# thiviyanT/torch-rgcn

Measured on AMD Instinct MI355X. Metric: edges/s/GPU (fwd+bwd) 2-layer RGCN, 1M nodes/10M edges/50 rels, h=16, higher is better.
Workload: dtype f32; 1 GPU; S1: N=1000000 nodes, E=10000000 base triples, R0=50 relations (layer R=101), M=21000000 messages/layer, hidden=16, 2 NC layers (horizontal, vertical), fwd+bwd, learnable X

## Files before the change

### torch-rgcn_amd/csrc/rgcn_bwd_own.hip

```cpp
#include <stdlib.h>
#include <string.h>

#include <algorithm>

#include "rgcn_device.h"

namespace {

constexpr int OWN_REC = 176;
constexpr int OWN_REC_ROWS = 128;
constexpr int OWN_REC_HDR = 160;
constexpr int OWN_LDS_MAX = 160 * 1024;
#ifndef RGCN_OWN_NW
#define RGCN_OWN_NW 16
#define RGCN_OWN_K 8
#define RGCN_OWN_U 2
#endif
constexpr int OWN_NW = RGCN_OWN_NW;
constexpr int OWN_K = RGCN_OWN_K;
constexpr int OWN_U = RGCN_OWN_U;
constexpr int OWN_MAX_ROWS = (OWN_LDS_MAX - OWN_NW * BW_SCR2 * 4 - 64) / 192;

#define OWN_DW_CASE(I)                                                                                             \
  if constexpr (I < K) {                                                                                           \
    if (lr == I) {                                                                                                 \
      _Pragma("unroll") for (int t4 = 0; t4 < 4; ++t4)                                                             \
        accw[I] = __builtin_amdgcn_mfma_f32_16x16x4f32(a[t4], b[t4], accw[I], 0, 0, 0);                            \
    }                                                                                                              \
    asm volatile("" : "+s"(lr));                                                                                   \
  }

size_t bwd_own_lds(int rows, bool packed = false) { return (size_t)rows * 192 + (size_t)OWN_NW * BW_SCR2 * 4 + 64 + (packed ? PK_LDS : 0); }
constexpr int OWN_MAX_ROWS_PK = (OWN_LDS_MAX - OWN_NW * BW_SCR2 * 4 - 64 - PK_LDS) / 192;

template <bool RELU, int NW, int K, int ABL = 0, bool BF = false, bool PK = false>
__global__ __launch_bounds__(64 * NW) void bwd_own_d16_kernel(
    const float *__restrict__ G, const float *__restrict__ X, const float *__restrict__ Wtp, float *__restrict__ dX,
    float *__restrict__ dWout, const char *__restrict__ rec, const int *__restrict__ gptr, int gstride, int shared_rel, int n_tiles,
    int tile_rows, int n_dst, float *__restrict__ dbias, int n_src, const int *__restrict__ unit_rel) {
  constexpr int U = OWN_U, NT = 64 * NW;
  constexpr int TQ = (OWN_MAX_ROWS * 4 + NT - 1) / NT;
  static_assert(K <= 9, "dw_add lists nine accumulator cases");
  extern __shared__ __attribute__((aligned(16))) char lds[];
  const int tid = threadIdx.x;
  const int wave = __builtin_amdgcn_readfirstlane(tid >> 6), lane = tid & 63;
  const unsigned xt_off = (unsigned)tile_rows * 128u;
  const unsigned xs_off = (unsigned)tile_rows * 192u;
  float4 *dxz = reinterpret_cast<float4 *>(lds);
  const double2 *dxd2 = reinterpret_cast<const double2 *>(lds);
  float4 *xt4 = reinterpret_cast<float4 *>(lds + xt_off);
  float *xs = reinterpret_cast<float *>(lds + xs_off) + wave * BW_SCR2;
  int *ctr = reinterpret_cast<int *>(lds + xs_off + (unsigned)NW * BW_SCR2 * 4u);
  const bool takes = shared_rel >= 0 && __builtin_amdgcn_readfirstlane(unit_rel[wave * K + K - 1]) == shared_rel;
  auto take = [&]() {
    int v = 0;
    if (lane == 0) v = __hip_atomic_fetch_add(ctr, U, __ATOMIC_RELAXED, __HIP_MEMORY_SCOPE_WORKGROUP);
    return __builtin_amdgcn_readfirstlane(v);
  };
  auto ranges = [&](int tt, int &a, int &b, int &sa, int &sb) {
    const int *g = gptr + (size_t)tt * gstride;
    a = __builtin_amdgcn_readfirstlane(g[wave]);
    b = __builtin_amdgcn_readfirstlane(g[wave + 1]);
    sa = sb = 0;
    if (takes) {
      sa = __builtin_amdgcn_readfirstlane(g[NW]);
      sb = __builtin_amdgcn_readfirstlane(g[NW + 1]);
    }
  };

  int t = blockIdx.x;
  int row0 = t * tile_rows;
  int nrows = min(tile_rows, n_dst - row0);
  int c0, c1, s0, s1;
  ranges(t, c0, c1, s0, s1);
  if (tid == 0) lds_st(ctr, 0);
  const float *dict = reinterpret_cast<const float *>(ctr + 16);
  if constexpr (PK)
    for (int i = tid; i <= PK_DICT; i += NT) ctr[16 + i] = i < PK_DICT ? reinterpret_cast<const int *>(rec)[i] : 0;
  float4 gs = make_float4(0.f, 0.f, 0.f, 0.f);
  const long long g_n4 = dbias ? (long long)n_src * 4 : 0, g_step = (long long)gridDim.x * NT;
  long long g_i = (long long)blockIdx.x * NT + tid;
#pragma unroll
  for (int q = 0; q < TQ; ++q) {
    const int idx = tid + q * NT;
    if (idx < tile_rows * 4) {
      float4 x0 = make_float4(0.f, 0.f, 0.f, 0.f);
      if (idx < nrows * 4) {
        if constexpr (BF) x0 = bf16x4_widen(reinterpret_cast<const uint2 *>(X)[(size_t)row0 * 4 + idx]);
        else x0 = reinterpret_cast<const float4 *>(X + (size_t)row0 * 16)[idx];
      }
      xt4[idx] = x0;
    }
  }
  for (int i = tid; i < tile_rows * 8; i += NT) dxz[i] = make_float4(0.f, 0.f, 0.f, 0.f);
  __syncthreads();

  const int m = lane & 15, k = lane >> 4;
  const unsigned kofs = (unsigned)k << 4;
  const unsigned dx_lane = (unsigned)m * 8u;
  const unsigned xrd = xt_off + (unsigned)m * 4u;
  float *xs_wr = xs + m * 16 + 4 * ((k + (m >> 2)) & 3);
  const float *xs_rd = xs + (4 * k) * 16 + 4 * (((m >> 2) + k) & 3) + (m & 3);
  const unsigned slot_lane = (unsigned)m * 8u;
  const unsigned rows_lane = (unsigned)OWN_REC_ROWS + (unsigned)k * 8u;
  const unsigned w_lane = (unsigned)lane * 16u;

  f32x4 accw[K];
#pragma unroll
  for (int i = 0; i < K; ++i) accw[i] = f32x4{0.f, 0.f, 0.f, 0.f};
  auto dw_add = [&](int lr, const float (&a)[4], const float (&b)[4]) {
    OWN_DW_CASE(0) OWN_DW_CASE(1) OWN_DW_CASE(2) OWN_DW_CASE(3) OWN_DW_CASE(4) OWN_DW_CASE(5) OWN_DW_CASE(6) OWN_DW_CASE(7) OWN_DW_CASE(8)
  };

  uint2 sl_n[U], rw_n[U];
  int hd_n[U];
  auto request_idx = [&](int c, int last) {
#pragma unroll
    for (int j = 0; j < U; ++j) {
      const int cc = min(c + j, last);
      if constexpr (PK) {
        const char *r = rec + PK_DICT_BYTES + (size_t)cc * PK_REC;
        sl_n[j].x = *reinterpret_cast<const unsigned *>(r + (unsigned)m * 4u);
        rw_n[j] = *reinterpret_cast<const uint2 *>(r + ((unsigned)PK_REC_ROWS + (unsigned)k * 8u));
      } else {
      const char *r = rec + (size_t)cc * OWN_REC;
      sl_n[j] = *reinterpret_cast<const uint2 *>(r + slot_lane);
      rw_n[j] = *reinterpret_cast<const uint2 *>(r + rows_lane);
      hd_n[j] = *reinterpret_cast<const int *>(r + OWN_REC_HDR);
      }
    }
  };
  if (c0 < c1) request_idx(c0, c1 - 1);

  for (;;) {
    int c = c0, last = c1 - 1;
    bool sh = false;
    if (c > last && s0 < s1) {
      sh = true;
      c = s0 + take();
      last = s1 - 1;
      if (c <= last) request_idx(c, last);
    }
    while (c <= last) {
      unsigned w0_[U];
      uint2 rw_[U];
      float v_[U];
      int hd_[U];
      float4 g_[U], w_[U];
#pragma unroll
      for (int j = 0; j < U; ++j) {
        if constexpr (PK) {
          w0_[j] = (sl_n[j].x >> 2) & 0xFFFFFFC0u;
          rw_[j] = rw_n[j];
          v_[j] = dict[(c + j <= last) ? sl_n[j].x & 0xFFu : (unsigned)PK_DICT];
          hd_[j] = pk_header(__builtin_amdgcn_readfirstlane(rw_n[j].x), __builtin_amdgcn_readfirstlane(rw_n[j].y));
        } else {
        w0_[j] = sl_n[j].x;
        rw_[j] = rw_n[j];
        v_[j] = (c + j <= last) ? __builtin_bit_cast(float, sl_n[j].y) : 0.f;
        hd_[j] = __builtin_amdgcn_readfirstlane(hd_n[j]);
        }
      }
      if constexpr (PK) {
#pragma unroll
        for (int j = 0; j < U; ++j) asm volatile("" : "+v"(w0_[j]));
      } else {
#pragma unroll
      for (int j = 0; j < U; ++j) asm volatile("" : "+v"(w0_[j]), "+v"(v_[j]));
      }
      __builtin_amdgcn_sched_barrier(0);
#pragma unroll
      for (int j = 0; j < U; ++j) {
        if constexpr (BF) {
          g_[j] = bf16x4_widen(*reinterpret_cast<const uint2 *>(reinterpret_cast<const char *>(G) + ((w0_[j] >> 1) | (kofs >> 1))));
        } else {
          const unsigned og = w0_[j] | kofs;
          g_[j] = *reinterpret_cast<const float4 *>(reinterpret_cast<const char *>(G) + og);
        }
        w_[j] = *reinterpret_cast<const float4 *>(reinterpret_cast<const char *>(Wtp) + (size_t)(hd_[j] & 0xFFFF) * 1024 + w_lane);
      }
      __builtin_amdgcn_sched_barrier(0);
      {
        int cn = c + U, lastn = last;
        if (sh || (cn > last && s0 < s1)) {
          sh = true;
          cn = s0 + take();
          lastn = s1 - 1;
        }
        if (cn <= lastn) request_idx(cn, lastn);
        c = cn;
        last = lastn;
      }
      __builtin_amdgcn_sched_barrier(0);
      if (ABL & 16) {
#pragma unroll
        for (int j = 0; j < U; ++j) asm volatile("" :: "v"(g_[j].x), "v"(g_[j].y), "v"(g_[j].z), "v"(g_[j].w), "v"(w_[j].x), "v"(w_[j].w), "v"(rw_[j].x), "v"(rw_[j].y), "v"(v_[j]));
        continue;
      }
      f32x4 sc[U], acc[U];
#pragma unroll
      for (int j = 0; j < U; ++j) {
        sc[j] = f32x4{g_[j].x * v_[j], g_[j].y * v_[j], g_[j].z * v_[j], g_[j].w * v_[j]};
        acc[j] = f32x4{0.f, 0.f, 0.f, 0.f};
      }
#pragma unroll
      for (int j = 0; j < U; ++j) acc[j] = __builtin_amdgcn_mfma_f32_16x16x4f32(sc[j][0], w_[j].x, acc[j], 0, 0, 0);
#pragma unroll
      for (int j = 0; j < U; ++j) acc[j] = __builtin_amdgcn_mfma_f32_16x16x4f32(sc[j][1], w_[j].y, acc[j], 0, 0, 0);
#pragma unroll
      for (int j = 0; j < U; ++j) acc[j] = __builtin_amdgcn_mfma_f32_16x16x4f32(sc[j][2], w_[j].z, acc[j], 0, 0, 0);
#pragma unroll
      for (int j = 0; j < U; ++j) acc[j] = __builtin_amdgcn_mfma_f32_16x16x4f32(sc[j][3], w_[j].w, acc[j], 0, 0, 0);
      unsigned ro[U][4];
#pragma unroll
      for (int j = 0; j < U; ++j) {
        ro[j][0] = rw_[j].x & 0xFFFFu;
        ro[j][1] = rw_[j].x >> 16;
        ro[j][2] = rw_[j].y & 0xFFFFu;
        ro[j][3] = rw_[j].y >> 16;
        if constexpr (PK) {
#pragma unroll
          for (int e = 0; e < 4; ++e) ro[j][e] &= 0xFFC0u;
        }
      }
#pragma unroll
      for (int h = 0; h < U && !(ABL & 2); h += 2) {
        constexpr int P = 2;
        float bv[P][4], av[P][4];
#pragma unroll
        for (int jj = 0; jj < P; ++jj) {
          const int j = h + jj;
          if (j >= U) break;
          asm volatile("" ::: "memory");
          *reinterpret_cast<f32x4 *>(xs_wr) = sc[j];
          asm volatile("" ::: "memory");
#pragma unroll
          for (int t4 = 0; t4 < 4; ++t4) bv[jj][t4] = xs_rd[16 * t4];
#pragma unroll
          for (int t4 = 0; t4 < 4; ++t4) av[jj][t4] = *reinterpret_cast<const float *>(lds + (xrd + ro[j][t4]));
          asm volatile("" ::: "memory");
        }
#pragma unroll
        for (int jj = 0; jj < P; ++jj) {
          if (h + jj >= U) break;
          dw_add((int)((unsigned)hd_[h + jj] >> 16), av[jj], bv[jj]);
        }
      }
#pragma unroll
      for (int j = 0; j < U && !(ABL & 8); ++j)
#pragma unroll
        for (int e = 0; e < 4; ++e)
          __hip_atomic_fetch_add(static_cast<double *>(__builtin_assume_aligned(lds + (dx_lane + 2u * ro[j][e]), 8)), (double)acc[j][e], __ATOMIC_RELAXED,
                                 __HIP_MEMORY_SCOPE_WORKGROUP);
      __builtin_amdgcn_sched_barrier(0);
    }
    const int tn = t + (int)gridDim.x;
    int c0n = 0, c1n = 0, s0n = 0, s1n = 0, row0n = 0, nrn = 0;
    float4 xn[TQ];
#pragma unroll
    for (int q = 0; q < TQ; ++q) xn[q] = make_float4(0.f, 0.f, 0.f, 0.f);
    if (tn < n_tiles) {
      row0n = tn * tile_rows;
      nrn = min(tile_rows, n_dst - row0n);
      ranges(tn, c0n, c1n, s0n, s1n);
#pragma unroll
      for (int q = 0; q < TQ; ++q)
        if (tid + q * NT < nrn * 4) {
          if constexpr (BF) {
            const uint2 u = reinterpret_cast<const uint2 *>(X)[(size_t)row0n * 4 + tid + q * NT];
            xn[q] = make_float4(__uint_as_float(u.x), __uint_as_float(u.y), 0.f, 0.f);
          } else {
            xn[q] = reinterpret_cast<const float4 *>(X + (size_t)row0n * 16)[tid + q * NT];
          }
        }
      if (c0n < c1n) request_idx(c0n, c1n - 1);
    }
    float4 gn = make_float4(0.f, 0.f, 0.f, 0.f);
    if (g_i < g_n4) {
      if constexpr (BF) gn = bf16x4_widen(reinterpret_cast<const uint2 *>(G)[g_i]);
      else gn = reinterpret_cast<const float4 *>(G)[g_i];
    }
    g_i += g_step;
    lds_barrier();
    gs.x += gn.x; gs.y += gn.y; gs.z += gn.z; gs.w += gn.w;
#pragma unroll
    for (int q = 0; q < TQ; ++q) asm volatile("" : "+v"(xn[q].x), "+v"(xn[q].y), "+v"(xn[q].z), "+v"(xn[q].w));
#pragma unroll
    for (int q = 0; q < TQ; ++q) {
      const int idx = tid + q * NT;
      if (idx < nrows * 4) {
        const double2 d0 = dxd2[2 * idx], d1 = dxd2[2 * idx + 1];
        float4 a = make_float4((float)d0.x, (float)d0.y, (float)d1.x, (float)d1.y);
        if (RELU) {
          const float4 x = xt4[idx];
          a.x = x.x > 0.f ? a.x : 0.f; a.y = x.y > 0.f ? a.y : 0.f; a.z = x.z > 0.f ? a.z : 0.f; a.w = x.w > 0.f ? a.w : 0.f;
        }
        if constexpr (BF) reinterpret_cast<uint2 *>(dX)[(size_t)row0 * 4 + idx] = bf16x4_round(a);
        else reinterpret_cast<float4 *>(dX + (size_t)row0 * 16)[idx] = a;
      }
    }
    if (tn >= n_tiles) break;
    if (tid == 0) lds_st(ctr, 0);
#pragma unroll
    for (int q = 0; q < TQ; ++q) {
      const int idx = tid + q * NT;
      if (idx < tile_rows * 4) {
        dxz[2 * idx] = make_float4(0.f, 0.f, 0.f, 0.f);
        dxz[2 * idx + 1] = make_float4(0.f, 0.f, 0.f, 0.f);
        if constexpr (BF) xt4[idx] = bf16x4_widen(uint2{__float_as_uint(xn[q].x), __float_as_uint(xn[q].y)});
        else xt4[idx] = xn[q];
      }
    }
    lds_barrier();
    t = tn; row0 = row0n; nrows = nrn; c0 = c0n; c1 = c1n; s0 = s0n; s1 = s1n;
  }
  if (dbias) {
    for (; g_i < g_n4; g_i += g_step) {
      float4 gn;
      if constexpr (BF) gn = bf16x4_widen(reinterpret_cast<const uint2 *>(G)[g_i]);
      else gn = reinterpret_cast<const float4 *>(G)[g_i];
      gs.x += gn.x; gs.y += gn.y; gs.z += gn.z; gs.w += gn.w;
    }
#pragma unroll
    for (int sft = 4; sft < 64; sft <<= 1) {
      gs.x += __shfl_xor(gs.x, sft); gs.y += __shfl_xor(gs.y, sft); gs.z += __shfl_xor(gs.z, sft); gs.w += __shfl_xor(gs.w, sft);
    }
    __syncthreads();
    if (lane < 4) *reinterpret_cast<float4 *>(xs + 4 * lane) = gs;
    __syncthreads();
    if (tid < 16) {
      float a = 0.f;
      const float *all = reinterpret_cast<const float *>(lds + xs_off);
      for (int i = 0; i < NW; ++i) a += all[i * BW_SCR2 + tid];
      atomicAdd(dbias + tid, a);
    }
  }
  if (shared_rel >= 0) {
    __syncthreads();
    *reinterpret_cast<f32x4 *>(xs + 4 * lane) = takes ? accw[K - 1] : f32x4{0.f, 0.f, 0.f, 0.f};
    __syncthreads();
    if (wave == 0) {
      const float *all = reinterpret_cast<const float *>(lds + xs_off) + 4 * lane;
      f32x4 a = f32x4{0.f, 0.f, 0.f, 0.f};
      for (int i = 0; i < NW; ++i) a += *reinterpret_cast<const f32x4 *>(all + i * BW_SCR2);
      float *o = dWout + (size_t)shared_rel * 256 + (4 * k) * 16 + m;
      atomicAdd(o, a[0]);
      atomicAdd(o + 16, a[1]);
      atomicAdd(o + 32, a[2]);
      atomicAdd(o + 48, a[3]);
    }
  }
#pragma unroll
  for (int li = 0; li < K; ++li) {
    const int r = __builtin_amdgcn_readfirstlane(unit_rel[wave * K + li]);
    if (r >= 0 && !(takes && li == K - 1)) {
      float *o = dWout + (size_t)r * 256 + (4 * k) * 16 + m;
      atomicAdd(o, accw[li][0]);
      atomicAdd(o + 16, accw[li][1]);
      atomicAdd(o + 32, accw[li][2]);
      atomicAdd(o + 48, accw[li][3]);
    }
  }
}

#undef OWN_DW_CASE

}

extern "C" int32_t rgcn_bwd_own_waves(void) { return OWN_NW; }
extern "C" int32_t rgcn_bwd_own_units(void) { return OWN_NW * OWN_K; }
extern "C" int32_t rgcn_bwd_own_max_rows(void) { return OWN_MAX_ROWS; }
extern "C" int32_t rgcn_bwd_blk_packed_max_rows(int32_t owner) { return owner ? OWN_MAX_ROWS_PK : rgcn_spmm_blk_max_rows(); }

static bool own_groups_ok(const int32_t *own_ptr, const int32_t *group_ptr, int32_t shared_rel, int64_t n_tiles, int32_t R) {
  if (!group_ptr) return own_ptr && shared_rel < 0;
  return shared_rel >= 0 && shared_rel < R && n_tiles * (int64_t)(OWN_NW + 1) < INT32_MAX;
}

extern "C" int rgcn_bwd_own_f32(const float *G, const float *X, const float *Wt_packed, float *dX, float *dW, const void *rec,
                                const int32_t *own_ptr, const int32_t *group_ptr, int32_t shared_rel, const int32_t *unit_rel, int64_t n_tiles,
                                int32_t tile_rows, int64_t n_dst, int32_t R, int32_t flags, float *dbias, int64_t n_src, void *stream) {
  if (!G || !X || !Wt_packed || !dX || !dW || !rec || !unit_rel || n_tiles <= 0 || tile_rows <= 0 || n_dst <= 0 || R <= 0 ||
      R > 0xFFFF || n_dst > INT32_MAX || n_tiles * (int64_t)OWN_NW >= INT32_MAX || !own_groups_ok(own_ptr, group_ptr, shared_rel, n_tiles, R)) {
    rgcn_set_error("bwd_own: bad argument");
    return RGCN_EINVAL;
  }
  const bool packed = (flags & RGCN_F_PACKED_REC) != 0;
  if (tile_rows > (packed ? OWN_MAX_ROWS_PK : OWN_MAX_ROWS)) {
    rgcn_set_error("bwd_own: tiles of at most %d rows (got %d)", packed ? OWN_MAX_ROWS_PK : OWN_MAX_ROWS, tile_rows);
    return RGCN_EUNSUPPORTED;
  }
  if (n_src <= 0 || n_src >= (int64_t(1) << 26)) {
    rgcn_set_error("bwd_own: the records address G rows as src << 6 in 32 bits: 0 < n_src < 2^26");
    return RGCN_EINVAL;
  }
  hipStream_t st = (hipStream_t)stream;
  int dev = 0, n_cu = 0;
  HIP_TRY(launch_device(&dev, &n_cu));
  HIP_TRY(zero_dw_dbias_async(dW, (size_t)R, dbias, st));
  const size_t lds = bwd_own_lds(tile_rows, packed);
  const unsigned n_blocks = (unsigned)std::min<int64_t>(n_tiles, n_cu);
  auto launch = [&](auto k) -> hipError_t {
    constexpr auto kern = decltype(k)::value;
    hipError_t e = allow_lds<kern>(dev, lds, OWN_LDS_MAX);
    if (e != hipSuccess) return e;
    hipLaunchKernelGGL(kern, dim3(n_blocks), dim3(64 * OWN_NW), lds, st, G, X, Wt_packed, dX, dW, static_cast<const char *>(rec), group_ptr ? group_ptr : own_ptr,
                       group_ptr ? OWN_NW + 1 : OWN_NW, group_ptr ? shared_rel : -1, (int)n_tiles, tile_rows, (int)n_dst, dbias, (int)n_src, unit_rel);
    return hipGetLastError();
  };
#ifdef RGCN_ABLATIONS
  {
    const int ABLV = rgcn_option_value(RGCN_OPT_BWD_ABL);
    if (packed) { rgcn_set_error("bwd_own (ablation library): wide records only"); return RGCN_EUNSUPPORTED; }
    if (ABLV == 2) HIP_TRY(launch(kern_c<bwd_own_d16_kernel<false, OWN_NW, OWN_K, 2>>));
    else if (ABLV == 8) HIP_TRY(launch(kern_c<bwd_own_d16_kernel<false, OWN_NW, OWN_K, 8>>));
    else if (ABLV == 16) HIP_TRY(launch(kern_c<bwd_own_d16_kernel<false, OWN_NW, OWN_K, 16>>));
    else HIP_TRY(launch(kern_c<bwd_own_d16_kernel<false, OWN_NW, OWN_K, 0>>));
    return RGCN_OK;
  }
#endif
  if (packed && (flags & RGCN_F_RELU)) HIP_TRY(launch(kern_c<bwd_own_d16_kernel<true, OWN_NW, OWN_K, 0, false, true>>));
  else if (packed) HIP_TRY(launch(kern_c<bwd_own_d16_kernel<false, OWN_NW, OWN_K, 0, false, true>>));
  else if (flags & RGCN_F_RELU) HIP_TRY(launch(kern_c<bwd_own_d16_kernel<true, OWN_NW, OWN_K>>));
  else HIP_TRY(launch(kern_c<bwd_own_d16_kernel<false, OWN_NW, OWN_K>>));
  return RGCN_OK;
}

extern "C" int rgcn_bwd_own_bf16(const uint16_t *G, const uint16_t *X, const float *Wt_packed, uint16_t *dX, float *dW, const void *rec,
                                 const int32_t *own_ptr, const int32_t *group_ptr, int32_t shared_rel, const int32_t *unit_rel, int64_t n_tiles,
                                 int32_t tile_rows, int64_t n_dst, int32_t R, int32_t flags, float *dbias, int64_t n_src, void *stream) {
  if (!G || !X || !Wt_packed || !dX || !dW || !rec || !unit_rel || n_tiles <= 0 || tile_rows <= 0 || n_dst <= 0 || R <= 0 ||
      R > 0xFFFF || n_dst > INT32_MAX || n_tiles * (int64_t)OWN_NW >= INT32_MAX || n_src <= 0 || n_src >= (int64_t(1) << 26) || (flags & ~RGCN_F_PACKED_REC) != 0 ||
      !own_groups_ok(own_ptr, group_ptr, shared_rel, n_tiles, R)) {
    rgcn_set_error("bwd_own_bf16: bad argument (the records address G rows as src << 6 in 32 bits: n_src < 2^26; no flags)");
    return RGCN_EINVAL;
  }
  const bool packed = (flags & RGCN_F_PACKED_REC) != 0;
  if (tile_rows > (packed ? OWN_MAX_ROWS_PK : OWN_MAX_ROWS)) {
    rgcn_set_error("bwd_own_bf16: tiles of at most %d rows (got %d)", packed ? OWN_MAX_ROWS_PK : OWN_MAX_ROWS, tile_rows);
    return RGCN_EUNSUPPORTED;
  }
  hipStream_t st = (hipStream_t)stream;
  int dev = 0, n_cu = 0;
  HIP_TRY(launch_device(&dev, &n_cu));
  HIP_TRY(zero_dw_dbias_async(dW, (size_t)R, dbias, st));
  const size_t lds = bwd_own_lds(tile_rows, packed);
  const unsigned n_blocks = (unsigned)std::min<int64_t>(n_tiles, n_cu);
  auto launch = [&](auto k) -> hipError_t {
    constexpr auto kern = decltype(k)::value;
    hipError_t e = allow_lds<kern>(dev, lds, OWN_LDS_MAX);
    if (e != hipSuccess) return e;
    hipLaunchKernelGGL(kern, dim3(n_blocks), dim3(64 * OWN_NW), lds, st, reinterpret_cast<const float *>(G), reinterpret_cast<const float *>(X),
                       Wt_packed, reinterpret_cast<float *>(dX), dW, static_cast<const char *>(rec), group_ptr ? group_ptr : own_ptr,
                       group_ptr ? OWN_NW + 1 : OWN_NW, group_ptr ? shared_rel : -1, (int)n_tiles, tile_rows, (int)n_dst, dbias, (int)n_src, unit_rel);
    return hipGetLastError();
  };
  if (packed) HIP_TRY(launch(kern_c<bwd_own_d16_kernel<false, OWN_NW, OWN_K, 0, true, true>>));
  else HIP_TRY(launch(kern_c<bwd_own_d16_kernel<false, OWN_NW, OWN_K, 0, true>>));
  return RGCN_OK;
}
```

### torch-rgcn_amd/torch_rgcn/graph.py

```python
import numpy as np
import torch

from . import _native, routes

_LDS_WAVE_FLOATS = 2048


def pick_tile_rows(width, n_rows=None):
    ld = (max(1, width) + 3) & ~3
    env = routes.get("tile_rows")
    if env:
        return max(1, min(int(env), 4096 // ld))
    rows = max(1, min(128, _LDS_WAVE_FLOATS // ld))
    if n_rows is not None and n_rows < rows * 2048:
        rows = max(min(rows, 8), min(rows, n_rows // 2048))
    return int(rows)


_MAX_CELLS = 2 ** 34
_SOFTWIN_MIN_CHUNKS = 4
_OWN_MAX_IMBALANCE = 1.25


class RelGraph:
    def __init__(self, triples_plus, val, num_nodes, num_rels, device):
        self.num_nodes, self.num_rels = int(num_nodes), int(num_rels)
        self.device = torch.device(device)
        if self.device.type != "cuda":
            raise RuntimeError("RelGraph lives on a GPU: torch_rgcn runs on HIP kernels only (no CPU fallback)")
        if self.num_nodes * self.num_rels >= _MAX_CELLS:
            raise NotImplementedError(f"num_nodes * num_relations = {self.num_nodes * self.num_rels:,} needs a "
                                      f"{4 * self.num_nodes * self.num_rels / 2**30:.0f} GiB counting table (limit {_MAX_CELLS:,} cells)")
        self._dev = None
        self._plans = {}
        self.perm = self.inv = None
        self.sync_free = False
        self.per_call = False
        self.owned_relations = None
        if triples_plus is None:
            return
        tp = np.ascontiguousarray(triples_plus, dtype=np.int64).reshape(-1, 3)
        self._s = tp[:, 0].astype(np.int32)
        self._p = tp[:, 1].astype(np.int32)
        self._o = tp[:, 2].astype(np.int32)
        self._val = np.ascontiguousarray(val, dtype=np.float32)
        self.num_messages = tp.shape[0]

    @classmethod
    def on_device(cls, s, p, o, val, alive, n_live, num_nodes, num_rels):
        g = cls(None, None, num_nodes, num_rels, s.device)
        g._dev = (s, p, o, val, alive)
        g.num_messages = int(n_live)
        return g

    def _plan(self, kind, tile_rows, max_item_chunks=64):
        whole = routes.get("deterministic", "0") == "1"
        key = (kind, tile_rows, max_item_chunks, whole)
        if key not in self._plans and self._dev is not None:
            N, R = self.num_nodes, self.num_rels
            s, p, o, val, alive = self._dev
            dst, src = (s, o) if kind == "fwd" else (o, s)
            nosync = self.sync_free or self.per_call
            self._plans[key] = _native.build_plan_device(dst, src, p, val, alive, N, N, R, tile_rows, self.num_messages,
                                                         max_item_chunks, want_runs=True, want_pack=True, sync_free=nosync,
                                                         **({"max_unit_chunks": 1 << 30} if whole else {}))
        if key not in self._plans:
            N, R = self.num_nodes, self.num_rels
            if kind == "fwd":
                hp = _native.build_plan_host(self._s, self._o, self._p, self._val, N, N, R, tile_rows, max_item_chunks,
                                             want_runs=True, want_pack=True, **({"max_unit_chunks": 1 << 30} if whole else {}))
            elif kind == "bwd":
                hp = _native.build_plan_host(self._o, self._s, self._p, self._val, N, N, R, tile_rows, max_item_chunks,
                                             want_runs=True, want_pack=True, **({"max_unit_chunks": 1 << 30} if whole else {}))
            else:
                raise KeyError(kind)
            self._plans[key] = _native.DevicePlan(hp, self.device)
        return self._plans[key]

    def fwd_plan(self, d_out):
        return self._plan("fwd", pick_tile_rows(d_out, self.num_nodes))

    def bwd_plan(self, d_in):
        rows = pick_tile_rows(d_in, self.num_nodes)
        if d_in == 16 and not routes.is_set("tile_rows"):
            rows = min(rows, 64)
        return self._plan("bwd", rows)

    def bwd_blk_plan(self, diag4=False, sparse=False, rows=None):
        if routes.is_set("tile_rows"):
            return None
        if rows is None:
            rows = _native.bwd_blk_rows(self.num_nodes, self.num_rels, routes.get("deterministic", "0") == "1", self.device, diag4,
                                        sparse)
        return self._plan("bwd", rows) if rows else None

    def fwd_blk_plan(self):
        if routes.is_set("tile_rows"):
            return None
        rows = _native.spmm_blk_rows(self.num_nodes, self.device)
        if not rows:
            return None
        plan = self._plan("fwd", rows)
        return plan if plan.run_ptr is not None and plan.n_src < (1 << 26) else None

    def win_plan(self, kind, rows=None):
        if routes.get("softwin", "auto") == "0" or routes.get("deterministic", "0") == "1" or routes.is_set("tile_rows") or \
                self._dev is None or self.sync_free or self.per_call:
            return None
        if rows is None:
            rows = _native.bwd_own_rows(self.num_nodes, self.device) if kind == "bwd_own" else _native.spmm_blk_rows(self.num_nodes, self.device)
        if not rows or self.num_nodes >= (1 << 26):
            return None
        n_tiles = -(-self.num_nodes // rows)
        if routes.get("softwin", "auto") != "1" and \
                self.num_messages < _SOFTWIN_MIN_CHUNKS * 16 * n_tiles * self.num_rels:
            return None
        key = ("win", kind, rows)
        if key not in self._plans:
            s, p, o, val, alive = self._dev
            dst, src = (s, o) if kind == "fwd" else (o, s)
            own = {}
            if kind == "bwd_own":
                nw, per_wave, max_rows = _native.bwd_own_geometry()
                if rows > max_rows or self.num_rels > nw * per_wave:
                    self._plans[key] = None
                    return None
                own = {"own_waves": nw, "own_per_wave": per_wave, "own_shared": True}
            plan = _native.build_softwin_plan(dst, src, p, val, alive, self.num_nodes, self.num_nodes, self.num_rels, rows, **own)
            if plan is not None and own and plan.own_balance > _OWN_MAX_IMBALANCE:
                plan = None
            self._plans[key] = plan
        return self._plans[key]

    def wgt_plan(self):
        return self._plan("fwd", max(self.num_nodes, 1), int(routes.get("wgrad_item_chunks", "64")))

    def csr(self, kind, need_slot=False):
        key = ("csr", kind)
        if key in self._plans and need_slot and self._plans[key].msg_slot is None:
            del self._plans[key]
        if key not in self._plans:
            if self._dev is None:
                raise RuntimeError("the basis-aggregation path needs the device-side graph build")
            s, p, o, val, alive = self._dev
            if self.per_call and not need_slot and ("csr", "fwd") not in self._plans \
                    and ("csr", "bwd") not in self._plans:
                self._plans[("csr", "fwd")], self._plans[("csr", "bwd")] = \
                    _native.build_csr_pair_device(s, o, p, val, alive, self.num_nodes)
                return self._plans[key]
            dst, src = (s, o) if kind == "fwd" else (o, s)
            self._plans[key] = _native.build_csr_device(dst, src, p, val, alive, self.num_nodes, sync_free=self.sync_free,
                                                        want_slot=need_slot or not self.per_call)
            self._plans[key].per_call = self.per_call
            self._plans[key].num_rels = self.num_rels
        return self._plans[key]

    def fbasis_plan(self):
        if "fbasis" not in self._plans:
            self._plans["fbasis"] = _native.build_fbasis_plan(self.csr("bwd"), self.csr("fwd"), self.num_nodes, self.num_rels)
        return self._plans["fbasis"]

    def max_degree(self):
        if self.sync_free:
            return 0
        if "maxdeg" not in self._plans:
            m = 0
            for kind in ("fwd", "bwd"):
                rp = self.csr(kind).rowptr
                m = max(m, int((rp[1:] - rp[:-1]).max().item()) if rp.numel() > 1 else 0)
            self._plans["maxdeg"] = m
        return self._plans["maxdeg"]

    def scatter_plan(self, kind, item_chunks=64):
        key = ("scatter", kind, item_chunks)
        if key not in self._plans:
            if self._dev is None:
                raise RuntimeError("the relation-major two-pass paths need the device-side graph build")
            s, p, o, val, alive = self._dev
            dst, src = (s, o) if kind == "fwd" else (o, s)
            csr = self.csr(kind, need_slot=True)
            if csr.n_messages is None:
                csr.n_messages = int(csr.rowptr[-1].item())
            N, R = self.num_nodes, self.num_rels
            self._plans[key] = _native.build_plan_device(dst, src, p, val, alive, N, N, R, max(N, 1), self.num_messages,
                                                         item_chunks, aux=csr.msg_slot)
        return self._plans[key]

    def selfloop_edges(self, self_rel):
        if self._dev is not None:
            s, p, o, val, alive = self._dev
            m = p == self_rel
            if alive is not None:
                m = m & (alive != 0)
            return s[m].long(), o[m].long(), val[m]
        m = self._p == self_rel
        dev = self.device
        return (torch.from_numpy(self._s[m].astype(np.int64)).to(dev), torch.from_numpy(self._o[m].astype(np.int64)).to(dev),
                torch.from_numpy(self._val[m]).to(dev))


def _device_build_enabled():
    return routes.get("graph_build", "device") == "device"


def node_order(s, o, num_nodes, how):
    s = np.asarray(s, dtype=np.int64)
    o = np.asarray(o, dtype=np.int64)
    if how == "degree":
        deg = np.bincount(s, minlength=num_nodes) + np.bincount(o, minlength=num_nodes)
        order = np.argsort(-deg, kind="stable")
    elif how in ("rcm", "bfs"):
        import scipy.sparse as sp
        from scipy.sparse import csgraph
        keep = s != o
        A = sp.coo_matrix((np.ones(int(keep.sum()), np.int8), (s[keep], o[keep])), shape=(num_nodes, num_nodes)).tocsr()
        A = ((A + A.T) > 0).astype(np.int8).tocsr()
        if how == "rcm":
            order = np.asarray(csgraph.reverse_cuthill_mckee(A, symmetric_mode=True), dtype=np.int64)
        else:
            deg = np.asarray(A.sum(axis=1)).ravel()
            seen = np.zeros(num_nodes, bool)
            parts = []
            for start in np.argsort(-deg, kind="stable"):
                if seen[start]:
                    continue
                comp = csgraph.breadth_first_order(A, int(start), directed=False, return_predecessors=False)
                seen[comp] = True
                parts.append(comp)
                if seen.all():
                    break
            order = np.concatenate(parts).astype(np.int64)
    else:
        raise NotImplementedError(f"node order {how!r} (degree, rcm, bfs)")
    perm = np.empty(num_nodes, dtype=np.int64)
    perm[order] = np.arange(num_nodes, dtype=np.int64)
    return perm


_AUTO_MIN_NODES = 500_000
_AUTO_HUB_SHARE = 0.30


def _auto_order(s, o, num_nodes):
    if num_nodes < _AUTO_MIN_NODES or s.numel() == 0:
        return "none"
    deg = torch.bincount(s.long(), minlength=num_nodes) + torch.bincount(o.long(), minlength=num_nodes)
    top = max(1, num_nodes // 100)
    share = deg.topk(top).values.sum().item() / max(1, int(deg.sum().item()))
    return "degree" if share >= _AUTO_HUB_SHARE else "none"


def graph_from_nc_triples(triples_plus, num_nodes, num_rels, vertical, device, relabel=None):
    relabel = relabel if relabel is not None else (routes.get("relabel") or "auto")
    if _device_build_enabled() and num_nodes * num_rels < _MAX_CELLS:
        t = torch.as_tensor(triples_plus, dtype=torch.long).reshape(-1, 3).to(device)
        M = t.shape[0]
        n_swap = int((M - num_nodes) / 2)
        assert vertical or (n_swap >= 0 and 2 * n_swap + num_nodes == M), \
            f"edge_norm: horizontal swap needs 2n+i == M (n={n_swap} i={num_nodes} M={M})"
        s, p, o, err = _native.dev_split_triples(t, num_nodes, num_rels)
        _native.dev_check_err(err, "stack_matrices")
        val = _native.dev_edge_norm(s, p, o, None, num_nodes, num_rels, vertical, max(n_swap, 0))
        perm = None
        if relabel == "auto":
            relabel = _auto_order(s, o, num_nodes)
        if relabel and relabel != "none":
            perm = torch.from_numpy(node_order(s.cpu().numpy(), o.cpu().numpy(), num_nodes, relabel)).to(device)
            p32 = perm.to(torch.int32)
            s, o = p32[s.long()].contiguous(), p32[o.long()].contiguous()
        g = RelGraph.on_device(s, p, o, val, None, M, num_nodes, num_rels)
        if perm is not None:
            g.perm = perm
            g.inv = torch.empty_like(perm)
            g.inv[perm] = torch.arange(num_nodes, device=perm.device)
        return g
    tp = triples_plus.detach().cpu().numpy() if torch.is_tensor(triples_plus) else np.asarray(triples_plus)
    tp = np.ascontiguousarray(tp, dtype=np.int64).reshape(-1, 3)
    M = tp.shape[0]
    val = _native.edge_norm_host(tp, num_nodes, num_rels, vertical, int((M - num_nodes) / 2), num_nodes)
    return RelGraph(tp, val, num_nodes, num_rels, device)


def graph_from_lp_triples(triples, num_nodes, num_rels, vertical, keep_mask, device):
    if _device_build_enabled() and num_nodes * num_rels < _MAX_CELLS:
        t = torch.as_tensor(triples, dtype=torch.long).reshape(-1, 3).to(device)
        E = t.shape[0]
        s, p, o, alive, err = _native.dev_lp_expand(t, num_nodes, (num_rels - 1) // 2, keep_mask)
        _native.dev_check_err(err, "stack_matrices")
        val = _native.dev_edge_norm(s, p, o, alive, num_nodes, num_rels, vertical, E)
        sync_free = _native._deferred_mode()
        n_live = 3 * E + num_nodes
        g = RelGraph.on_device(s, p, o, val, alive, n_live, num_nodes, num_rels)
        g.sync_free = sync_free
        g.per_call = True
        return g
    t = triples.detach().cpu().numpy() if torch.is_tensor(triples) else np.asarray(triples)
    t = np.ascontiguousarray(t, dtype=np.int64).reshape(-1, 3)
    R0 = (num_rels - 1) // 2
    keep = None if keep_mask is None else keep_mask.detach().cpu().numpy().astype(np.uint8)
    tp, n_self = _native.lp_augment_host(t, num_nodes, R0, keep)
    val = _native.edge_norm_host(tp, num_nodes, num_rels, vertical, t.shape[0], n_self)
    return RelGraph(tp, val, num_nodes, num_rels, device)
```

### torch-rgcn_amd/torch_rgcn/routes.py

```python
import contextlib
import os

NAMES = (
    "deterministic", "relabel", "tile_rows", "bwd", "bwd_kernel", "twopass", "featureless_csr", "dist_comm", "dist_slabs", "deferred_checks",
    "block_path", "block_fwd", "wgrad_tiles", "wgrad_item_chunks", "wgrad", "spmm_csr", "sparse_path", "graph_build", "fbasis_inplace_mb", "fbasis",
    "distmult_bwd", "diag_path", "capture", "fbasis_tile", "pad16_view", "softwin", "softwin_build", "bwd_own", "own_rows_cap",
    "packed_rec",
)
NATIVE = ("bwd_nw", "gemm_bm", "spmm_u", "wgrad_rg", "wgrad_u", "bwd_abl")

_values = {}
_native_sink = None


def _seed():
    _values.clear()
    for n in NAMES + NATIVE:
        v = os.environ.get("RGCN_" + n.upper())
        if v is not None and v != "":
            _values[n] = v


_seed()


def get(name, default=None):
    assert name in NAMES or name in NATIVE, f"unknown route {name!r}"
    return _values.get(name, default)


def is_set(name):
    return get(name) is not None


def flag(name, default=False):
    v = get(name)
    return default if v is None else v == "1"


def push_native(name=None):
    if _native_sink is None:
        return
    for n in ((name,) if name else NATIVE):
        v = _values.get(n)
        _native_sink(n, None if v is None else int(v))


def set(name, value):
    assert name in NAMES or name in NATIVE, f"unknown route {name!r}"
    if value is None:
        _values.pop(name, None)
    else:
        _values[name] = str(value)
    if name in NATIVE:
        push_native(name)


@contextlib.contextmanager
def override(**kw):
    saved = {k: _values.get(k) for k in kw}
    try:
        for k, v in kw.items():
            set(k, v)
        yield
    finally:
        for k, v in saved.items():
            set(k, v)


def patch(monkeypatch, name, value):
    assert name in NAMES or name in NATIVE, f"unknown route {name!r}"
    if value is None:
        monkeypatch.delitem(_values, name, raising=False)
    else:
        monkeypatch.setitem(_values, name, str(value))
    if name in NATIVE:
        push_native(name)


def snapshot():
    return dict(_values)
```

Measured before the change: 7.082 billion edges/s.

## Generalize owner-kernel weight-gradient flush to merge any relation shared across waves

Replaces the single shared_rel block reduction in the owner backward kernel with a general scheme. A per-block table of the waves' relation assignments is built, and DPP comparisons within 16-lane rows precompute which unit slots hold a relation duplicated across waves. For those slots the waves reduce through LDS and only the first owning wave issues the atomics; other slots flush directly. A new own_level option, off by default, is passed to the plan builder, presumably to allow relation splitting across waves. This adds per-slot barriers where duplicates exist.

```diff
diff --git a/torch-rgcn_amd/csrc/rgcn_bwd_own.hip b/torch-rgcn_amd/csrc/rgcn_bwd_own.hip
--- a/torch-rgcn_amd/csrc/rgcn_bwd_own.hip
+++ b/torch-rgcn_amd/csrc/rgcn_bwd_own.hip
@@ -30,6 +30,12 @@
     asm volatile("" : "+s"(lr));                                                                                   \
   }
 
+template <int J>
+__device__ __forceinline__ bool own_row_dup(int v) {
+  if constexpr (J == 16) return false;
+  else return (v == __builtin_amdgcn_update_dpp(0, v, 0x120 + J, 0xF, 0xF, false)) | own_row_dup<J + 1>(v);
+}
+
 size_t bwd_own_lds(int rows, bool packed = false) { return (size_t)rows * 192 + (size_t)OWN_NW * BW_SCR2 * 4 + 64 + (packed ? PK_LDS : 0); }
 constexpr int OWN_MAX_ROWS_PK = (OWN_LDS_MAX - OWN_NW * BW_SCR2 * 4 - 64 - PK_LDS) / 192;
 
@@ -41,6 +47,7 @@
   constexpr int U = OWN_U, NT = 64 * NW;
   constexpr int TQ = (OWN_MAX_ROWS * 4 + NT - 1) / NT;
   static_assert(K <= 9, "dw_add lists nine accumulator cases");
+  static_assert(NW <= 16, "the flush compares the waves' relations inside one row of 16 lanes");
   extern __shared__ __attribute__((aligned(16))) char lds[];
   const int tid = threadIdx.x;
   const int wave = __builtin_amdgcn_readfirstlane(tid >> 6), lane = tid & 63;
@@ -68,6 +75,27 @@
     }
   };
 
+  constexpr int KQ = (K + 3) / 4;
+  auto own_table = [&](int (&tb)[KQ], int ln) {
+#pragma unroll
+    for (int q = 0; q < KQ; ++q) {
+      const int li = 4 * q + (ln >> 4), w = ln & 15;
+      tb[q] = (li < K && w < NW) ? unit_rel[w * K + li] : -1;
+    }
+  };
+  unsigned cutmask = 0;
+  {
+    int tb[KQ];
+    own_table(tb, lane);
+#pragma unroll
+    for (int q = 0; q < KQ; ++q) {
+      const unsigned long long d = __ballot(tb[q] >= 0 && own_row_dup<1>(tb[q]));
+#pragma unroll
+      for (int j = 0; j < 4; ++j) cutmask |= ((d >> (16 * j)) & 0xFFFFull) ? 1u << (4 * q + j) : 0u;
+    }
+    cutmask = __builtin_amdgcn_readfirstlane(cutmask);
+  }
+
   int t = blockIdx.x;
   int row0 = t * tile_rows;
   int nrows = min(tile_rows, n_dst - row0);
@@ -314,6 +342,9 @@
     lds_barrier();
     t = tn; row0 = row0n; nrows = nrn; c0 = c0n; c1 = c1n; s0 = s0n; s1 = s1n;
   }
+  int tab[KQ], ln = lane;
+  asm volatile("" : "+v"(ln));
+  own_table(tab, ln);
   if (dbias) {
     for (; g_i < g_n4; g_i += g_step) {
       float4 gn;
@@ -328,6 +359,8 @@
     __syncthreads();
     if (lane < 4) *reinterpret_cast<float4 *>(xs + 4 * lane) = gs;
     __syncthreads();
+#pragma unroll
+    for (int q = 0; q < KQ; ++q) asm volatile("" : "+v"(tab[q]));
     if (tid < 16) {
       float a = 0.f;
       const float *all = reinterpret_cast<const float *>(lds + xs_off);
@@ -335,30 +368,34 @@
       atomicAdd(dbias + tid, a);
     }
   }
-  if (shared_rel >= 0) {
-    __syncthreads();
-    *reinterpret_cast<f32x4 *>(xs + 4 * lane) = takes ? accw[K - 1] : f32x4{0.f, 0.f, 0.f, 0.f};
-    __syncthreads();
-    if (wave == 0) {
-      const float *all = reinterpret_cast<const float *>(lds + xs_off) + 4 * lane;
-      f32x4 a = f32x4{0.f, 0.f, 0.f, 0.f};
-      for (int i = 0; i < NW; ++i) a += *reinterpret_cast<const f32x4 *>(all + i * BW_SCR2);
-      float *o = dWout + (size_t)shared_rel * 256 + (4 * k) * 16 + m;
+#pragma unroll
+  for (int li = 0; li < K; ++li) {
+    const int row = tab[li >> 2];
+    const int r = __builtin_amdgcn_readlane(row, 16 * (li & 3) + wave);
+    f32x4 a = accw[li];
+    bool flush = r >= 0;
+    if ((cutmask >> li) & 1u) {
+      const unsigned same = r >= 0 ? (unsigned)(__ballot(row == r) >> (16 * (li & 3))) & 0xFFFFu : 0u;
+      lds_barrier();
+      *reinterpret_cast<f32x4 *>(xs + 4 * lane) = accw[li];
+      lds_barrier();
+      flush = r >= 0 && (same & ((1u << wave) - 1u)) == 0u;
+      if (flush) {
+        const float *all = reinterpret_cast<const float *>(lds + xs_off) + 4 * lane;
+        a = f32x4{0.f, 0.f, 0.f, 0.f};
+#pragma unroll 4
+        for (int i = 0; i < NW; ++i) {
+          const f32x4 v = *reinterpret_cast<const f32x4 *>(all + i * BW_SCR2);
+          if ((same >> i) & 1u) a += v;
+        }
+      }
+    }
+    if (flush) {
+      float *o = dWout + (size_t)r * 256 + (4 * k) * 16 + m;
       atomicAdd(o, a[0]);
       atomicAdd(o + 16, a[1]);
       atomicAdd(o + 32, a[2]);
       atomicAdd(o + 48, a[3]);
-    }
-  }
-#pragma unroll
-  for (int li = 0; li < K; ++li) {
-    const int r = __builtin_amdgcn_readfirstlane(unit_rel[wave * K + li]);
-    if (r >= 0 && !(takes && li == K - 1)) {
-      float *o = dWout + (size_t)r * 256 + (4 * k) * 16 + m;
-      atomicAdd(o, accw[li][0]);
-      atomicAdd(o + 16, accw[li][1]);
-      atomicAdd(o + 32, accw[li][2]);
-      atomicAdd(o + 48, accw[li][3]);
     }
   }
 }
diff --git a/torch-rgcn_amd/torch_rgcn/graph.py b/torch-rgcn_amd/torch_rgcn/graph.py
--- a/torch-rgcn_amd/torch_rgcn/graph.py
+++ b/torch-rgcn_amd/torch_rgcn/graph.py
@@ -20,6 +20,7 @@
 _MAX_CELLS = 2 ** 34
 _SOFTWIN_MIN_CHUNKS = 4
 _OWN_MAX_IMBALANCE = 1.25
+_OWN_LEVEL = False
 
 
 class RelGraph:
@@ -125,7 +126,7 @@
                 if rows > max_rows or self.num_rels > nw * per_wave:
                     self._plans[key] = None
                     return None
-                own = {"own_waves": nw, "own_per_wave": per_wave, "own_shared": True}
+                own = {"own_waves": nw, "own_per_wave": per_wave, "own_shared": True, "own_level": routes.flag("own_level", _OWN_LEVEL)}
             plan = _native.build_softwin_plan(dst, src, p, val, alive, self.num_nodes, self.num_nodes, self.num_rels, rows, **own)
             if plan is not None and own and plan.own_balance > _OWN_MAX_IMBALANCE:
                 plan = None
diff --git a/torch-rgcn_amd/torch_rgcn/routes.py b/torch-rgcn_amd/torch_rgcn/routes.py
--- a/torch-rgcn_amd/torch_rgcn/routes.py
+++ b/torch-rgcn_amd/torch_rgcn/routes.py
@@ -5,7 +5,7 @@
     "deterministic", "relabel", "tile_rows", "bwd", "bwd_kernel", "twopass", "featureless_csr", "dist_comm", "dist_slabs", "deferred_checks",
     "block_path", "block_fwd", "wgrad_tiles", "wgrad_item_chunks", "wgrad", "spmm_csr", "sparse_path", "graph_build", "fbasis_inplace_mb", "fbasis",
     "distmult_bwd", "diag_path", "capture", "fbasis_tile", "pad16_view", "softwin", "softwin_build", "bwd_own", "own_rows_cap",
-    "packed_rec",
+    "packed_rec", "own_level",
 )
 NATIVE = ("bwd_nw", "gemm_bm", "spmm_u", "wgrad_rg", "wgrad_u", "bwd_abl")
 
```

Result: no change. 7.075 billion edges/s (-0.1%).
